# VincentGourbin/ltx-video-swift-mlx

Hardware: AMD Instinct MI355X
Metric: DiT denoise steps/sec + VAE decode ms, 768x512x25 distilled (higher is better)
Workload: dtype bf16; 1 GPU; distilled 8-step schedule, 768x512x25 -> latent 4x16x24 (1536 tokens), 1024 text keys, CFG off, batch 1 per GPU, 48-layer DiT bf16 weights (random init); text_keys=1024, parallelism=replica x1 (one sample per GPU, no data-path collective)

## Files before the change

### include/ltxhip.h

```cpp
#ifndef LTXHIP_H
#define LTXHIP_H

#include <stddef.h>
#include <stdint.h>

#ifdef __cplusplus
extern "C" {
#endif

typedef struct ltx_ctx ltx_ctx;

typedef enum ltx_status {
    LTX_OK = 0,
    LTX_ERR_MODEL_NOT_LOADED = 1,
    LTX_ERR_INVALID_CONFIGURATION = 2,
    LTX_ERR_INSUFFICIENT_MEMORY = 3,
    LTX_ERR_WEIGHT_LOADING_FAILED = 4,
    LTX_ERR_GENERATION_FAILED = 5,
    LTX_ERR_GENERATION_CANCELLED = 6,
    LTX_ERR_INVALID_FRAME_COUNT = 7,
    LTX_ERR_INVALID_DIMENSIONS = 8,
    LTX_ERR_FILE_NOT_FOUND = 9,
    LTX_ERR_INVALID_LORA = 10,
    LTX_ERR_HIP = 11
// ... 333 lines not shown
                                const float* noise, int tile, int overlap, int root, float* frames_out, long frames_cap,
                                int* n_frames_out);

int ltx_prof_enable(ltx_ctx* ctx, int on);
int ltx_prof_collect(ltx_ctx* ctx, int kind, double* total_ms, long* launches, double* work, int reset);

int ltx_op_gemm_bf16(ltx_ctx* ctx, const uint16_t* A, long lda, const uint16_t* B, long ldb, const float* bias, int M,
                     int N, int K, int act, int tile_cfg, float* out_f32, long ld_f32, uint16_t* out_bf16,
                     long ld_bf16);
int ltx_op_gemm_q8(ltx_ctx* ctx, const uint16_t* A, long lda, const uint8_t* codes, const uint16_t* scales, const uint16_t* biases,
                   const float* bias, int M, int N, int K, int split_k, int via_scratch, int tile_cfg, float* out_f32, long ld_f32);
int ltx_op_value_projection_t(ltx_ctx* ctx, const uint16_t* X, long ldx, int tokens, const uint16_t* W, const float* bias, int out_features,
                              int in_features, uint16_t* vt, long ldvt);
int ltx_op_qkv_projection(ltx_ctx* ctx, const uint16_t* X, long ldx, int rows, int rows_per_batch, const uint16_t* Wqk, const float* bqk,
                          const uint16_t* Wv, const float* bv, int D, int K, uint16_t* qk_out, long ld_qk, uint16_t* vt_out, long ldvt,
                          int fused);
int ltx_op_gemm_bf16_gated_residual(ltx_ctx* ctx, const uint16_t* A, long lda, const uint16_t* B, long ldb,
                                    const float* bias, const float* gate, float gate_scalar, int M, int N, int K,
                                    float* x, long ldx, uint16_t* mirror_bf16, long ld_mirror);
int ltx_op_gemm_bf16_gated_residual_norm(ltx_ctx* ctx, const uint16_t* A, long lda, const uint16_t* B, long ldb,
                                         const float* bias, const float* gate, float gate_scalar, int M, int N, int K,
                                         float* x, long ldx, const float* scale, const float* shift, float eps,
                                         uint16_t* xn, long ldxn, int fused);
int ltx_op_gemv_f32(ltx_ctx* ctx, const float* a, long lda, const uint16_t* W, long ldw, const float* bias, float* out,
                    long ldo, int M, int N, int K, int in_act);
typedef struct ltx_gemv_job {
    const float* a;
    long lda;
    const uint16_t* W;
    long ldw;
    const float* bias;
    float* out;
    long ldo;
    int N;
    int K;
    int in_act;
} ltx_gemv_job;
int ltx_op_gemv_group(ltx_ctx* ctx, const ltx_gemv_job* jobs, int n_jobs, int M);
int ltx_op_attention(ltx_ctx* ctx, const uint16_t* Q, const uint16_t* K, const uint16_t* Vt, long ldvt,
                     const float* bias, int B, int H, int Tq, int Tk, float scale, uint16_t* O);
int ltx_attention_key_splits(int B, int H, int Tq, int Tk);
int ltx_op_attention_hd(ltx_ctx* ctx, const uint16_t* Q, const uint16_t* K, const uint16_t* Vt, long ldvt, const float* bias, int B, int H,
                        int Tq, int Tk, int head_dim, float scale, uint16_t* O);
int ltx_attention_hd_workgroup_queries(int B, int H, int Tq, int head_dim);
int ltx_op_norm_mod(ltx_ctx* ctx, const float* x, const float* scale, const float* shift, int rows, int D,
                    int norm_kind, float eps, int round_norm_bf16, uint16_t* out);
// ... 27 lines not shown
```

### ltx-video-swift-mlx_amd/__init__.py

```python
import contextlib
import ctypes as C

import numpy as np

from . import _lib
from ._lib import (ALLGATHER_FN, DIST_ID_BYTES, SHARD_CFG, SHARD_NONE, SHARD_SEQUENCE, ConnectorConfig, PROGRESS_CB, DenoiseOptions,
                   DualBlockConfig, DualDenoiseArgs, DualForwardArgs, DualModelConfig, DualModelForwardArgs, DualStepJob, GemvJob,
                   LTXError, NormMod2Job, TransformerConfig, lib)

__version__ = lib.ltx_version().decode()


def _check(rc, ctx=None):
    if rc != 0:
        msg = lib.ltx_last_error(ctx).decode(errors="replace") if True else ""
        raise LTXError(rc, msg)


def default_dual_block_config(**overrides):
    cfg = DualBlockConfig()
    lib.ltx_dual_block_config_default(C.byref(cfg))
    o = dict(overrides)
    if "video_heads" in o:
        o.setdefault("video_dim", o["video_heads"] * 128)
    if "audio_heads" in o:
        o.setdefault("audio_dim", o["audio_heads"] * 64)
    if "video_dim" in o:
        o.setdefault("video_context_dim", o["video_dim"])
    if "audio_dim" in o:
        o.setdefault("audio_context_dim", o["audio_dim"])
# ... 1008 lines not shown
```

### ltx-video-swift-mlx_amd/_lib.py

```python
import ctypes as C
import os

_HERE = os.path.dirname(os.path.abspath(__file__))
SO_PATH = os.environ.get("LTX_LIB") or os.path.join(_HERE, "csrc", "build", "libltxhip.so")


class LTXError(RuntimeError):

    NAMES = {
        1: "modelNotLoaded", 2: "invalidConfiguration", 3: "insufficientMemory", 4: "weightLoadingFailed",
        5: "generationFailed", 6: "generationCancelled", 7: "invalidFrameCount", 8: "invalidDimensions",
        9: "fileNotFound", 10: "invalidLoRA", 11: "hipError",
    }

    def __init__(self, code, message):
        self.code = int(code)
        self.case = self.NAMES.get(self.code, "unknown")
        super().__init__(f"LTXError.{self.case}: {message}")


class DenoiseOptions(C.Structure):

    _fields_ = [("struct_size", C.c_uint32), ("cfg_scale", C.c_float), ("guidance_rescale", C.c_float), ("stg_scale", C.c_float),
                ("stg_blocks", C.POINTER(C.c_int)), ("n_stg_blocks", C.c_int), ("ge_gamma", C.c_float),
# ... 22 lines not shown
        ("timestep_scale_multiplier", C.c_float), ("norm_eps", C.c_float),
    ]


class DualBlockConfig(C.Structure):

    _fields_ = [("num_layers", C.c_int), ("video_heads", C.c_int), ("video_dim", C.c_int), ("audio_heads", C.c_int), ("audio_dim", C.c_int),
                ("video_context_dim", C.c_int), ("audio_context_dim", C.c_int), ("rope_theta", C.c_float), ("max_pos", C.c_int * 3),
                ("audio_max_pos", C.c_int), ("fps", C.c_float), ("norm_eps", C.c_float)]


class DualForwardArgs(C.Structure):

    _fields_ = [("struct_size", C.c_uint32), ("B", C.c_int), ("F", C.c_int), ("H", C.c_int), ("W", C.c_int), ("T_a", C.c_int), ("S", C.c_int),
                ("x_video", C.c_void_p), ("x_audio", C.c_void_p), ("context_video", C.c_void_p), ("context_audio", C.c_void_p),
                ("key_bias_video", C.c_void_p), ("key_bias_audio", C.c_void_p), ("temb_video", C.c_void_p), ("temb_audio", C.c_void_p),
                ("cross_video_ss", C.c_void_p), ("cross_audio_ss", C.c_void_p), ("phase_mask", C.c_uint32)]


class GemvJob(C.Structure):

    _fields_ = [("a", C.c_void_p), ("lda", C.c_long), ("W", C.c_void_p), ("ldw", C.c_long), ("bias", C.c_void_p), ("out", C.c_void_p),
                ("ldo", C.c_long), ("N", C.c_int), ("K", C.c_int), ("in_act", C.c_int)]


class DualModelConfig(C.Structure):

    _fields_ = [("blocks", DualBlockConfig), ("in_channels", C.c_int), ("out_channels", C.c_int), ("audio_in_channels", C.c_int),
                ("audio_out_channels", C.c_int), ("caption_channels", C.c_int), ("timestep_scale_multiplier", C.c_float)]


class DualModelForwardArgs(C.Structure):

    _fields_ = [("struct_size", C.c_uint32), ("B", C.c_int), ("F", C.c_int), ("H", C.c_int), ("W", C.c_int), ("T_a", C.c_int), ("S", C.c_int),
                ("video_latent", C.c_void_p), ("audio_latent", C.c_void_p), ("video_context", C.c_void_p), ("audio_context", C.c_void_p),
                ("video_timesteps", C.c_void_p), ("audio_timesteps", C.c_void_p), ("video_mask", C.c_void_p), ("audio_mask", C.c_void_p),
                ("video_velocity", C.c_void_p), ("audio_velocity", C.c_void_p), ("ungrouped", C.c_int), ("text_cache", C.c_int)]


class NormMod2Job(C.Structure):

    _fields_ = [("x", C.c_void_p), ("ldx", C.c_long), ("scale0", C.c_void_p), ("shift0", C.c_void_p), ("scale1", C.c_void_p),
                ("shift1", C.c_void_p), ("mod_bstride", C.c_long), ("rows_per_batch", C.c_int), ("out0", C.c_void_p), ("out1", C.c_void_p),
                ("ldo", C.c_long), ("rows", C.c_int), ("D", C.c_int)]


# ... 143 lines not shown
    "ltx_audio_decode": (_i, [_vp, _vp, _i, _vp]),
    "ltx_audio_decode_dev": (_i, [_vp, _vp, _i, _vp]),
    "ltx_audio_latent_frames": (_i, [_i, _f]),
    "ltx_audio_mel_frames": (_i, [_i]),
    "ltx_audio_sample_count": (_l, [_i]),
    "ltx_audio_sample_rate": (_i, []),
    "ltx_write_wav": (_i, [C.c_char_p, _vp, _l, _i, _f]),
    "ltx_audio_positions": (_i, [_i, _vp]),
    "ltx_video_temporal_positions": (_i, [_i, _i, _i, _f, _vp]),
    "ltx_rope_tables_positions": (_i, [_vp, _i, _i, _f, _i, _vp, _vp]),
    "ltx_attn_module_init_synthetic": (_i, [_vp, _i, _i, _i, _i, _u64]),
    "ltx_attn_module_load": (_i, [_vp, _i, C.c_char_p, C.c_char_p, _i]),
    "ltx_attn_module_unload": (_i, [_vp, _i]),
    "ltx_attn_module_export_param": (_l, [_vp, _i, C.c_char_p, _vp, _l]),
    "ltx_attn_module_forward_dev": (_i, [_vp, _i, _vp, _vp, _i, _i, _i, _i, _vp, _vp, _i, _vp, _vp, _i, _vp, _vp]),
    "ltx_dual_block_config_default": (None, [C.POINTER(DualBlockConfig)]),
    "ltx_dual_blocks_init_synthetic": (_i, [_vp, C.POINTER(DualBlockConfig), _u64]),
    "ltx_dual_blocks_load": (_i, [_vp, C.c_char_p, C.POINTER(DualBlockConfig), _i, _i]),
    "ltx_dual_blocks_unload": (_i, [_vp]),
    "ltx_dual_blocks_export_param": (_l, [_vp, C.c_char_p, _vp, _l]),
    "ltx_dual_blocks_forward_dev": (_i, [_vp, C.POINTER(DualForwardArgs)]),
    "ltx_op_norm_mod2": (_i, [_vp, C.POINTER(NormMod2Job), C.POINTER(NormMod2Job), _f]),
    "ltx_op_gemv_group": (_i, [_vp, C.POINTER(GemvJob), _i, _i]),
    "ltx_dual_model_config_default": (None, [C.POINTER(DualModelConfig)]),
    "ltx_dual_model_init_synthetic": (_i, [_vp, C.POINTER(DualModelConfig), _u64]),
    "ltx_dual_model_load": (_i, [_vp, C.c_char_p, C.POINTER(DualModelConfig)]),
    "ltx_dual_model_unload": (_i, [_vp]),
    "ltx_dual_model_export_param": (_l, [_vp, C.c_char_p, _vp, _l]),
    "ltx_dual_model_forward_dev": (_i, [_vp, C.POINTER(DualModelForwardArgs)]),
    "ltx_dual_model_embed_dev": (_i, [_vp, _vp, _vp, _i, _i, _vp, _vp, _vp, _vp, _vp, _vp]),
    "ltx_dual_model_prepare_text_dev": (_i, [_vp, _vp, _vp, _vp, _vp, _i, _i]),
    "ltx_dual_model_text_cache_info": (_i, [_vp, _ip, _ip, C.POINTER(_l), C.POINTER(_l)]),
    "ltx_op_dual_step": (_i, [_vp, C.POINTER(DualStepJob), C.POINTER(DualStepJob), _f, _f]),
    "ltx_dual_denoise_dev": (_i, [_vp, C.POINTER(DualDenoiseArgs), PROGRESS_CB, _vp]),
    "ltx_dual_denoise": (_i, [_vp, C.POINTER(DualDenoiseArgs), PROGRESS_CB, _vp]),
    "ltx_op_attention_hd": (_i, [_vp, _vp, _vp, _vp, _l, _vp, _i, _i, _i, _i, _i, _f, _vp]),
    "ltx_attention_hd_workgroup_queries": (_i, [_i, _i, _i, _i]),
    "ltx_op_qknorm_rope_hd": (_i, [_vp, _vp, _l, _vp, _vp, _vp, _i, _i, _i, _i, _f, _f, _vp]),
    "ltx_op_conv1d": (_i, [_vp, _vp, _i, _i, _vp, _vp, _i, _i, _i, _i, _vp, _i, _i, _vp, _i, _f, _vp]),
    "ltx_op_conv_transpose1d": (_i, [_vp, _vp, _i, _i, _vp, _vp, _i, _i, _i, _i, _i, _vp, _i, _f, _vp]),
    "ltx_op_conv2d_causal": (_i, [_vp, _vp, _i, _i, _i, _vp, _vp, _i, _i, _i, _vp, _i, _vp, _vp]),
    "ltx_op_fill_normal_bf16": (_i, [_vp, _vp, _l, _u64, _f, _f]),
    "ltx_op_fill_normal_f32": (_i, [_vp, _vp, _l, _u64, _f, _f]),
}

for _name, (_res, _args) in SIGNATURES.items():
# ... 6 lines not shown
```

### ltx-video-swift-mlx_amd/csrc/abi_hooks.cpp

```cpp
#include <vector>

#include "abi_internal.h"
#include "attention.h"
#include "audio.h"
#include "elementwise.h"
#include "gemm.h"
#include "linear_ops.h"

namespace {

void op_workspace(ltx_ctx* ctx, size_t bytes) {
    if (ctx->op_ws.ensure(bytes)) HIP_CHECK(hipStreamSynchronize(ctx->stream));
}

const bf16_t* audio_halo_operand(ltx_ctx* ctx, const uint16_t* x, int Cin, int lines, int width, int pitch, size_t first, size_t total) {
    const size_t row = (size_t)Cin * 2;
    ctx->audio_op[0].ensure(total * row);
    char* base = ctx->audio_op[0].as<char>();
    if (pitch == width) {
        HIP_CHECK(hipMemsetAsync(base, 0, first * row, ctx->stream));
        const size_t end = first + (size_t)lines * width;
        HIP_CHECK(hipMemsetAsync(base + end * row, 0, (total - end) * row, ctx->stream));
        HIP_CHECK(hipMemcpyAsync(base + first * row, x, (size_t)lines * width * row, hipMemcpyDeviceToDevice, ctx->stream));
    } else {
// ... 151 lines not shown
                                         float* x, long ldx, const float* scale, const float* shift, float eps,
                                         uint16_t* xn, long ldxn, int fused) {
    return with_ctx(ctx, [&] {
        LTX_REQUIRE(A && B && x && scale && shift && xn, "ltx_op_gemm_bf16_gated_residual_norm: null argument");
        GemmArgs g;
        g.A = A; g.lda = lda; g.B = B; g.ldb = ldb; g.M = M; g.N = N; g.K = K;
        g.ep.bias_n = bias;
        g.ep.out_f32 = x; g.ep.ld_f32 = ldx;
        g.ep.resid = 1;
        g.ep.gate = gate; g.ep.gate_bstride = 0; g.ep.rows_per_batch = M; g.ep.gate_scalar = gate_scalar;
        op_workspace(ctx, (size_t)2 * M * N * 4);
        g.split_k = 0;
        g.split_ws = ctx->op_ws.as<float>();
        g.split_ws_elems = (long)(ctx->op_ws.bytes / 4);
        NormAfter na;
        na.scale = scale; na.shift = shift; na.mod_bstride = 0; na.rows_per_batch = M;
        na.out = xn; na.ldo = ldxn; na.eps = eps; na.norm_kind = LTX_NORM_RMS;
        if (fused) {
            launch_gemm_bf16(g, ctx->stream, &na);
        } else {
            launch_gemm_bf16(g, ctx->stream);
            launch_norm_mod(x, ldx, scale, shift, 0, M, xn, ldxn, M, N, LTX_NORM_RMS, eps, 0, ctx->stream);
        }
    });
}

int ltx_op_gemv_f32(ltx_ctx* ctx, const float* a, long lda, const uint16_t* W, long ldw, const float* bias, float* out,
                    long ldo, int M, int N, int K, int in_act) {
    return with_ctx(ctx, [&] { launch_gemv_f32(a, lda, W, ldw, bias, out, ldo, M, N, K, in_act, ctx->stream); });
}

int ltx_op_gemv_group(ltx_ctx* ctx, const ltx_gemv_job* jobs, int n_jobs, int M) {
    return with_ctx(ctx, [&] {
        LTX_REQUIRE(jobs && n_jobs >= 1 && n_jobs <= 8, "ltx_op_gemv_group: %d jobs out of range (1..8)", n_jobs);
        GemvJob g[8];
        for (int j = 0; j < n_jobs; ++j) {
            const ltx_gemv_job& q = jobs[j];
            g[j].a = q.a; g[j].lda = q.lda; g[j].W = q.W; g[j].ldw = q.ldw; g[j].bias = q.bias;
            g[j].out = q.out; g[j].ldo = q.ldo; g[j].N = q.N; g[j].K = q.K; g[j].in_act = q.in_act;
        }
        launch_gemv_group(g, n_jobs, M, ctx->stream);
    });
}

int ltx_op_conv3d(ltx_ctx* ctx, const uint16_t* x, int F, int H, int W, int Cin, const uint16_t* w, const float* bias,
                  int Cout, int causal, float* out) {
// ... 257 lines not shown
```

### ltx-video-swift-mlx_amd/csrc/gemm_asm_tiles.inc

```
namespace {

LTX_DEVFN int asm_src_offset(int lane, int wave, long ld) {
    const int srow = lane >> 3, pch = lane & 7;
    const int row0 = wave * 8 + srow;
    return (row0 * (int)ld + ((pch ^ ((row0 >> 1) & 7)) << 3)) * 2;
}
LTX_DEVFN uint32_t asm_src_stride(long ld) { return (uint32_t)(32 * ld * 2); }

struct AsmLane {
    int ao, bo;
    uint32_t sa, sb;
    uint32_t wlds;
    int fa0, fa1, fb0, fb1;
};
template <int WM, int WCOL, int A_BYTES>
LTX_DEVFN AsmLane asm_lane(int lane, int wave, int wr, int wc, long lda, long ldb) {
    AsmLane l;
    l.ao = asm_src_offset(lane, wave, lda);
    l.bo = asm_src_offset(lane, wave, ldb);
    l.sa = asm_src_stride(lda);
    l.sb = asm_src_stride(ldb);
    l.wlds = (uint32_t)wave * 1024u;
    const int frow = lane & 15, fsw = (lane >> 1) & 7;
    const int foff0 = frow * ROW_BYTES + ((((lane >> 4) + 0) ^ fsw) << 4);
    const int foff1 = frow * ROW_BYTES + ((((lane >> 4) + 4) ^ fsw) << 4);
    const int a_wave_off = (wr * WM) * ROW_BYTES, b_wave_off = 2 * A_BYTES + (wc * WCOL) * ROW_BYTES;
    l.fa0 = a_wave_off + foff0, l.fa1 = a_wave_off + foff1, l.fb0 = b_wave_off + foff0, l.fb1 = b_wave_off + foff1;
    return l;
}

struct AsmBufDesc {
    uint32_t lo, hi, rec;
};
LTX_DEVFN AsmBufDesc asm_buf_desc(const bf16_t* p, int rows, long ld, long kelems) {
    return {(uint32_t)(uintptr_t)p, (uint32_t)((uintptr_t)p >> 32), (uint32_t)(((long)(rows - 1) * ld + kelems) * 2)};
}

template <int WN>
LTX_DEVFN int asm_scratch_lane(int lane) { return (((lane >> 4) * 4) * WN + (lane & 15)) * 4; }

#if defined(DTL_STAMPS) || defined(QKV_STAMPS) || defined(TALL_STAMPS)
LTX_DEVFN unsigned long long* asm_stamp_slot(int wave) { return (blockIdx.x == 7) ? &g_gemm_stamps[wave][0] : &g_gemm_stamps[4][0]; }
#endif

LTX_DEVFN f32x4 asm_column_bias(const float* bias_n, int gn) { return bias_n ? *(const f32x4*)(bias_n + gn) : f32x4{0.f, 0.f, 0.f, 0.f}; }

template <bool BIAS_M>
LTX_DEVFN f32x4 asm_activate(const GemmEpilogue& ep, f32x4 v, int gm) {
    if constexpr (BIAS_M) {
        if (ep.bias_m) {
            const float bm = ep.bias_m[gm];
            v += f32x4{bm, bm, bm, bm};
        }
    }
    if (ep.act == LTX_ACT_GELU_TANH) {
#pragma unroll
        for (int e = 0; e < 4; ++e) v[e] = gelu_tanh(v[e]);
    } else if (ep.act == LTX_ACT_SILU) {
#pragma unroll
        for (int e = 0; e < 4; ++e) v[e] = silu_f(v[e]);
    }
    if (ep.round_bf16) {
#pragma unroll
        for (int e = 0; e < 4; ++e) v[e] = bf16_to_f32(f32_to_bf16(v[e]));
    }
// ... 8 lines not shown
LTX_DEVFN void asm_store(const GemmEpilogue& ep, int gm, int gn, const f32x4& v) {
    if (ep.out_f32) *(f32x4*)(ep.out_f32 + (long)gm * ep.ld_f32 + gn) = v;
    if (ep.out_bf16) asm_store_bf16(ep.out_bf16, ep.ld_bf16, gm, gn, v);
}
template <bool BIAS_M>
struct AsmPlainStore {
    const GemmEpilogue& ep;
    LTX_DEVFN void operator()(int gm, int gn, f32x4 v) const { asm_store(ep, gm, gn, asm_activate<BIAS_M>(ep, v, gm)); }
};

template <int WN>
struct AsmGroup {
    static constexpr int LPR = WN / 4, RPI = 64 / LPR, NITG = 32 / RPI;
};
template <int WN, class Put>
LTX_DEVFN void asm_store_group(const float* scr, int lane, int gm0, int gn, const f32x4& bias, Put&& put) {
    using G = AsmGroup<WN>;
    f32x4 vv[G::NITG];
#pragma unroll
    for (int it = 0; it < G::NITG; ++it) vv[it] = *(const f32x4*)(scr + (it * G::RPI + lane / G::LPR) * WN + (lane % G::LPR) * 4);
#pragma unroll
    for (int it = 0; it < G::NITG; ++it) put(gm0 + it * G::RPI + lane / G::LPR, gn, vv[it] + bias);
    asm volatile("s_waitcnt lgkmcnt(0)" ::: "memory");
}

__global__ __launch_bounds__(256, 1) void gemm_bf16_kernel_dtl(const GemmArgs g) {
    extern __shared__ __attribute__((aligned(16))) char smem[];
    constexpr int BM = 192, BN = 256, WGN = 2;
    constexpr int WM = 96, WN = 128;
    const int tid = threadIdx.x;
    const int lane = tid & 63;
    const int wave = __builtin_amdgcn_readfirstlane(tid >> 6);
    const int wr = wave / WGN, wc = wave % WGN;
    const int tiles_m = g.M / BM;
    const int bid = xcd_remap(blockIdx.x, gridDim.x);
    int tm, tn;
    tile_coords(g, bid, tiles_m, BN, tm, tn);
    const int m0 = tm * BM, n0 = tn * BN;
    int kt0 = 0, nkt = g.K / BK;
    if (g.split_k > 1) {
        const int z = blockIdx.y;
        kt0 = (int)((long)nkt * z / g.split_k);
        nkt = (int)((long)nkt * (z + 1) / g.split_k) - kt0;
    }
    const AsmLane l = asm_lane<WM, WN, BM * ROW_BYTES>(lane, wave, wr, wc, g.lda, g.ldb);
    const AsmBufDesc a = asm_buf_desc(g.A + (long)m0 * g.lda + (long)kt0 * BK, BM, g.lda, (long)nkt * BK);
    const AsmBufDesc b = asm_buf_desc(g.B + (long)n0 * g.ldb + (long)kt0 * BK, BN, g.ldb, (long)nkt * BK);
    const uint32_t nk = (uint32_t)nkt;
#ifdef DTL_STAMPS
    unsigned long long* dbg = asm_stamp_slot(wave);
#endif
    asm volatile(
#ifdef DTL_STAMPS
#include "gemm_dtl_192x256_stamps.inc"
#else
#include "gemm_dtl_192x256.inc"
#endif
        :
        : [alo] "s"(a.lo), [ahi] "s"(a.hi), [arec] "s"(a.rec), [blo] "s"(b.lo), [bhi] "s"(b.hi), [brec] "s"(b.rec), [nk] "s"(nk), [sa] "s"(l.sa),
          [sb] "s"(l.sb), [wlds] "s"(l.wlds), [ao] "v"(l.ao), [bo] "v"(l.bo), [fa0] "v"(l.fa0), [fa1] "v"(l.fa1), [fb0] "v"(l.fb0), [fb1] "v"(l.fb1)
#ifdef DTL_STAMPS
          , [dbg] "s"(dbg)
#endif
        :
#include "gemm_dtl_192x256_clobbers.inc"
    );
    __syncthreads();
    constexpr int LPR = AsmGroup<WN>::LPR, RPI = AsmGroup<WN>::RPI, NITG = AsmGroup<WN>::NITG;
    float* scr = (float*)(smem + wave * (32 * WN * 4));
    const unsigned scr_lane = (unsigned)(wave * (32 * WN * 4) + asm_scratch_lane<WN>(lane));
    const int gn = n0 + wc * WN + (lane % LPR) * 4;
    if (g.split_k > 1) {
        float* ws = g.split_ws + (long)blockIdx.y * g.M * g.N;
        bf16_t* wsb = (bf16_t*)g.split_ws + (long)blockIdx.y * g.M * g.N;
        static_for<0, 3>([&](auto grp_c) {
            constexpr int grp = decltype(grp_c)::value;
#include "gemm_asm_192x256_dump.inc"
#pragma unroll 4
            for (int it = 0; it < 32 / RPI; ++it) {
                const int row = it * RPI + lane / LPR;
                const f32x4 v = *(const f32x4*)(scr + row * WN + (lane % LPR) * 4);
                if (g.split_bf16) asm_store_bf16(wsb, g.N, m0 + wr * WM + grp * 32 + row, gn, v);
                else *(f32x4*)(ws + (long)(m0 + wr * WM + grp * 32 + row) * g.N + gn) = v;
            }
            asm volatile("s_waitcnt lgkmcnt(0)" ::: "memory");
        });
        return;
    }
    const GemmEpilogue& ep = g.ep;
    const f32x4 bias = asm_column_bias(ep.bias_n, gn);
    if (ep.resid) {
        const float* rbase = ep.resid_src ? ep.resid_src : ep.out_f32;
        const long rld = ep.resid_src ? ep.ld_resid : ep.ld_f32;
        const int row_lo = m0 + wr * WM, row_hi = row_lo + WM - 1;
        const bool gate_uniform = ep.gate && !ep.gate_rowmap && row_lo / ep.rows_per_batch == row_hi / ep.rows_per_batch;
        f32x4 gtu = f32x4{ep.gate_scalar, ep.gate_scalar, ep.gate_scalar, ep.gate_scalar};
        if (gate_uniform) gtu = *(const f32x4*)(ep.gate + (long)(row_lo / ep.rows_per_batch) * ep.gate_bstride + gn);
        f32x4 rs[2][NITG];
        auto fetch = [&](auto grp_c, auto buf_c) {
            constexpr int grp = decltype(grp_c)::value, buf = decltype(buf_c)::value;
#pragma unroll
            for (int it = 0; it < NITG; ++it) rs[buf][it] = *(const f32x4*)(rbase + (long)(m0 + wr * WM + grp * 32 + it * RPI + lane / LPR) * rld + gn);
        };
        fetch(std::integral_constant<int, 0>{}, std::integral_constant<int, 0>{});
        static_for<0, 3>([&](auto grp_c) {
            constexpr int grp = decltype(grp_c)::value;
            constexpr int buf = grp & 1;
            if constexpr (grp + 1 < 3) fetch(std::integral_constant<int, grp + 1>{}, std::integral_constant<int, (grp + 1) & 1>{});
#include "gemm_asm_192x256_dump.inc"
            static_for<0, 2>([&](auto half_c) {
                constexpr int half = decltype(half_c)::value;
                f32x4 vv[NITG / 2];
#pragma unroll
                for (int i2 = 0; i2 < NITG / 2; ++i2) vv[i2] = *(const f32x4*)(scr + ((half * (NITG / 2) + i2) * RPI + lane / LPR) * WN + (lane % LPR) * 4);
#pragma unroll
                for (int i2 = 0; i2 < NITG / 2; ++i2) {
                    const int it = half * (NITG / 2) + i2;
                    const int gm = m0 + wr * WM + grp * 32 + it * RPI + lane / LPR;
                    f32x4 v = asm_activate<true>(ep, vv[i2] + bias, gm);
                    f32x4 gt = gtu;
                    if (ep.gate && !gate_uniform)
                        gt = *(const f32x4*)(ep.gate + (long)(ep.gate_rowmap ? ep.gate_rowmap[gm] : gm / ep.rows_per_batch) * ep.gate_bstride + gn);
#pragma unroll
                    for (int e = 0; e < 4; ++e) v[e] = rs[buf][it][e] + gt[e] * v[e];
                    asm_store(ep, gm, gn, v);
                }
            });
            asm volatile("s_waitcnt lgkmcnt(0)" ::: "memory");
        });
        return;
    }
    static_for<0, 3>([&](auto grp_c) {
        constexpr int grp = decltype(grp_c)::value;
#include "gemm_asm_192x256_dump.inc"
        asm_store_group<WN>(scr, lane, m0 + wr * WM + grp * 32, gn, bias, AsmPlainStore<true>{ep});
    });
}

__global__ __launch_bounds__(256, 1) void gemm_bf16_kernel_qkv(const GemmQkvArgs g) {
    extern __shared__ __attribute__((aligned(16))) char smem[];
    constexpr int BM = 192, WM = 96, WNQ = 128, WNV = 64;
    const int tid = threadIdx.x;
    const int lane = tid & 63;
    const int wave = __builtin_amdgcn_readfirstlane(tid >> 6);
    const int wr = wave / 2, wc = wave % 2;
    const int tiles_m = g.M / BM;
    const int bid = xcd_remap(blockIdx.x, gridDim.x);
    int tm, tn;
    tile_coords(g.group_m, g.Nqk / 256, bid, tiles_m, tm, tn);
    const int m0 = tm * BM;
    const AsmLane l = asm_lane<WM, WNQ + WNV, BM * ROW_BYTES>(lane, wave, wr, wc, g.ldx, g.ldwqk);
    const int vo = asm_src_offset(lane, wave, g.ldwv);
    const uint32_t sv = asm_src_stride(g.ldwv);
    const AsmBufDesc a = asm_buf_desc(g.X + (long)m0 * g.ldx, BM, g.ldx, g.K);
    const AsmBufDesc b = asm_buf_desc(g.Wqk + (long)tn * 256 * g.ldwqk, 256, g.ldwqk, g.K);
    const AsmBufDesc v = asm_buf_desc(g.Wv + (long)tn * 128 * g.ldwv, 128, g.ldwv, g.K);
    const uint32_t nk = (uint32_t)(g.K / BK);
    constexpr int SPILL0 = 4 * 32 * WNQ * 4;
    const int sp = SPILL0 + wave * 8192 + lane * 16;
#ifdef QKV_STAMPS
    unsigned long long* dbg = asm_stamp_slot(wave);
#endif
    asm volatile(
#ifdef QKV_STAMPS
#include "gemm_qkv_192x384_stamps.inc"
#else
#include "gemm_qkv_192x384.inc"
#endif
        :
        : [alo] "s"(a.lo), [ahi] "s"(a.hi), [arec] "s"(a.rec), [blo] "s"(b.lo), [bhi] "s"(b.hi), [brec] "s"(b.rec), [vlo] "s"(v.lo), [vhi] "s"(v.hi),
          [vrec] "s"(v.rec), [nk] "s"(nk), [sa] "s"(l.sa), [sb] "s"(l.sb), [sv] "s"(sv), [wlds] "s"(l.wlds), [ao] "v"(l.ao), [bo] "v"(l.bo), [vo] "v"(vo),
          [fa0] "v"(l.fa0), [fa1] "v"(l.fa1), [fb0] "v"(l.fb0), [fb1] "v"(l.fb1), [sp] "v"(sp)
#ifdef QKV_STAMPS
          , [dbg] "s"(dbg)
#endif
        :
#include "gemm_qkv_192x384_clobbers.inc"
    );
    {
        const int bi = m0 / g.rows_per_batch;
        const int tok0 = m0 - bi * g.rows_per_batch + wr * WM + (lane >> 4) * 4;
        const int d0 = tn * 128 + wc * WNV + (lane & 15);
        bf16_t* vbase = g.vt + (long)bi * g.vt_bstride + tok0;
        float bv[4];
#pragma unroll
        for (int nv = 0; nv < 4; ++nv) bv[nv] = g.bias_v ? g.bias_v[d0 + nv * 16] : 0.f;
        static_for<0, 24>([&](auto vf_c) {
            constexpr int vf = decltype(vf_c)::value;
            constexpr int mi = vf / 4, nv = vf % 4;
            float f0, f1, f2, f3;
            if constexpr (vf < 16) {
#include "gemm_qkv_192x384_vread.inc"
            } else {
                const f32x4 t = *(const f32x4*)(smem + SPILL0 + wave * 8192 + (vf - 16) * 1024 + lane * 16);
                f0 = t[0], f1 = t[1], f2 = t[2], f3 = t[3];
            }
            const float bn = bv[nv];
            uint2 pk;
            pk.x = pack_bf16x2(f0 + bn, f1 + bn);
            pk.y = pack_bf16x2(f2 + bn, f3 + bn);
            *(uint2*)(vbase + (long)(d0 + nv * 16) * g.ldvt + mi * 16) = pk;
        });
    }
    constexpr int WN = WNQ;
    float* scr = (float*)(smem + wave * (32 * WN * 4));
    const unsigned scr_lane = (unsigned)(wave * (32 * WN * 4) + asm_scratch_lane<WN>(lane));
    const int gn = tn * 256 + wc * WN + (lane % AsmGroup<WN>::LPR) * 4;
    const f32x4 bias = asm_column_bias(g.bias_qk, gn);
    static_for<0, 3>([&](auto grp_c) {
        constexpr int grp = decltype(grp_c)::value;
#include "gemm_asm_192x256_dump.inc"
        asm_store_group<WN>(scr, lane, m0 + wr * WM + grp * 32, gn, bias,
                            [&](int gm, int gn_, const f32x4& val) { asm_store_bf16(g.qk, g.ld_qk, gm, gn_, val); });
    });
}

__global__ __launch_bounds__(256, 1) void gemm_bf16_kernel_tall(const GemmArgs g) {
    extern __shared__ __attribute__((aligned(16))) char smem[];
    constexpr int BM = 384, BN = 256, WGN = 2;
    constexpr int WM = 192, WN = 128;
    constexpr int WAVE_LDS = 2 * 32 * WN * 4;
    const int tid = threadIdx.x;
    const int lane = tid & 63;
    const int wave = __builtin_amdgcn_readfirstlane(tid >> 6);
    const int wr = wave / WGN, wc = wave % WGN;
    const int tiles_m = g.M / BM;
    const int bid = xcd_remap(blockIdx.x, gridDim.x);
    int tm, tn;
    tile_coords(g, bid, tiles_m, BN, tm, tn);
    const int m0 = tm * BM, n0 = tn * BN;
    const int nkt = g.K / BK;
    const AsmLane l = asm_lane<WM, WN, BM * ROW_BYTES>(lane, wave, wr, wc, g.lda, g.ldb);
    const AsmBufDesc a = asm_buf_desc(g.A + (long)m0 * g.lda, BM, g.lda, (long)nkt * BK);
    const AsmBufDesc b = asm_buf_desc(g.B + (long)n0 * g.ldb, BN, g.ldb, (long)nkt * BK);
    const uint32_t nk = (uint32_t)nkt;
    const int sp = wave * WAVE_LDS + asm_scratch_lane<WN>(lane);
#ifdef TALL_STAMPS
    unsigned long long* dbg = asm_stamp_slot(wave);
#endif
    asm volatile(
#ifdef TALL_STAMPS
#include "gemm_tall_384x256_stamps.inc"
#else
#include "gemm_tall_384x256.inc"
#endif
        :
        : [alo] "s"(a.lo), [ahi] "s"(a.hi), [arec] "s"(a.rec), [blo] "s"(b.lo), [bhi] "s"(b.hi), [brec] "s"(b.rec), [nk] "s"(nk), [sa] "s"(l.sa),
          [sb] "s"(l.sb), [wlds] "s"(l.wlds), [ao] "v"(l.ao), [bo] "v"(l.bo), [fa0] "v"(l.fa0), [fa1] "v"(l.fa1), [fb0] "v"(l.fb0), [fb1] "v"(l.fb1), [sp] "v"(sp)
#ifdef TALL_STAMPS
          , [dbg] "s"(dbg)
#endif
        :
#include "gemm_tall_384x256_clobbers.inc"
    );
    const unsigned scr_lane = (unsigned)(wave * WAVE_LDS + asm_scratch_lane<WN>(lane));
    const int gn = n0 + wc * WN + (lane % AsmGroup<WN>::LPR) * 4;
    const GemmEpilogue& ep = g.ep;
    const f32x4 bias = asm_column_bias(ep.bias_n, gn);
    static_for<0, 6>([&](auto ord_c) {
        constexpr int grp = (decltype(ord_c)::value + 4) % 6;
        const float* scr = (const float*)(smem + wave * WAVE_LDS + (grp == 5 ? 32 * WN * 4 : 0));
        if constexpr (grp < 4) {
#include "gemm_tall_384x256_dump.inc"
        }
        asm_store_group<WN>(scr, lane, m0 + wr * WM + grp * 32, gn, bias, AsmPlainStore<false>{ep});
    });
}

}

template <auto KERNEL, int SMEM, class Args>
static void launch_asm_tile(dim3 grid, const Args& a, hipStream_t stream) {
    static PerDeviceOnce attr_set;
    attr_set.run([&] { HIP_CHECK(hipFuncSetAttribute((const void*)KERNEL, hipFuncAttributeMaxDynamicSharedMemorySize, SMEM)); });
    hipLaunchKernelGGL(KERNEL, grid, dim3(256), SMEM, stream, a);
    HIP_CHECK(hipGetLastError());
}

static bool gemm_dtl_takes(const GemmArgs& a) {
    return !a.conv && a.M % 192 == 0 && a.N % 256 == 0 && a.K % 64 == 0 && a.K >= 64 && !a.ep.d2s && !a.ep.out_bf16_t &&
           a.lda % 8 == 0 && a.ldb % 8 == 0 && !a.ep.pn_out && !a.ep.clip01 && a.tile_count == 0 && a.win_rows == 0 &&
           (a.split_k <= 1 || (a.split_ws && a.split_k <= a.K / 64 && (long)a.split_k * a.M * a.N <= a.split_ws_elems));
}
static void launch_dtl(const GemmArgs& a, const GemmOpts& o, hipStream_t stream, const NormAfter* na = nullptr) {
    LTX_REQUIRE(gemm_dtl_takes(a), "gemm: the 192x256 kernel needs a dense A.B^T with M %% 192 == 0, N %% 256 == 0, K %% 64 == 0 (M=%d N=%d K=%d)",
                a.M, a.N, a.K);
    constexpr int smem = (2 * 192 + 3 * 256) * ROW_BYTES;
    launch_asm_tile<gemm_bf16_kernel_dtl, smem>(dim3((a.M / 192) * (a.N / 256), a.split_k > 1 ? a.split_k : 1), a, stream);
    if (a.split_k > 1) {
// ... 57 lines not shown
```

Before: 30.68 steps/s.

## Specialise asm GEMM epilogues with compile-time store variants and strength-reduced row pointers

Adds templated row-store functors that precompute output row pointers and step them by constant strides. A runtime variant selector dispatches common epilogues (plain bf16, GELU-tanh bf16, f32, f32+bf16 mirror, gated residual fast paths) to compile-time specialised loops, so the generic per-element epilogue branching is skipped. The same store path is applied to the DTL, QKV, tall and split-K partial kernels. It also adds optional epilogue cycle stamps and a standalone ltx_op_gemm_tile ABI entry for testing tiles, at the cost of more code and instantiations.

Result: faster. 31.19 steps/s (median of 6 runs) (+1.7%).

```diff
diff --git a/include/ltxhip.h b/include/ltxhip.h
--- a/include/ltxhip.h
+++ b/include/ltxhip.h
@@ -379,6 +379,34 @@
                                          const float* bias, const float* gate, float gate_scalar, int M, int N, int K,
                                          float* x, long ldx, const float* scale, const float* shift, float eps,
                                          uint16_t* xn, long ldxn, int fused);
+typedef struct ltx_gemm_tile_launch {
+    uint32_t struct_size;
+    int tile_cfg;
+    const uint16_t* A;
+    long lda;
+    const uint16_t* B;
+    long ldb;
+    int M, N, K;
+    int split_k;
+    int split_bf16;
+    int act;
+    int round_bf16;
+    int resid;
+    const float* bias_n;
+    const float* bias_m;
+    float* out_f32;
+    long ld_f32;
+    uint16_t* out_bf16;
+    long ld_bf16;
+    const float* resid_src;
+    long ld_resid;
+    const float* gate;
+    long gate_bstride;
+    const int32_t* gate_rowmap;
+    int rows_per_batch;
+    float gate_scalar;
+} ltx_gemm_tile_launch;
+int ltx_op_gemm_tile(ltx_ctx* ctx, const ltx_gemm_tile_launch* launch);
 int ltx_op_gemv_f32(ltx_ctx* ctx, const float* a, long lda, const uint16_t* W, long ldw, const float* bias, float* out,
                     long ldo, int M, int N, int K, int in_act);
 typedef struct ltx_gemv_job {
diff --git a/ltx-video-swift-mlx_amd/__init__.py b/ltx-video-swift-mlx_amd/__init__.py
--- a/ltx-video-swift-mlx_amd/__init__.py
+++ b/ltx-video-swift-mlx_amd/__init__.py
@@ -5,7 +5,7 @@
 
 from . import _lib
 from ._lib import (ALLGATHER_FN, DIST_ID_BYTES, SHARD_CFG, SHARD_NONE, SHARD_SEQUENCE, ConnectorConfig, PROGRESS_CB, DenoiseOptions,
-                   DualBlockConfig, DualDenoiseArgs, DualForwardArgs, DualModelConfig, DualModelForwardArgs, DualStepJob, GemvJob,
+                   DualBlockConfig, DualDenoiseArgs, DualForwardArgs, DualModelConfig, DualModelForwardArgs, DualStepJob, GemmTileLaunch, GemvJob,
                    LTXError, NormMod2Job, TransformerConfig, lib)
 
 __version__ = lib.ltx_version().decode()
diff --git a/ltx-video-swift-mlx_amd/_lib.py b/ltx-video-swift-mlx_amd/_lib.py
--- a/ltx-video-swift-mlx_amd/_lib.py
+++ b/ltx-video-swift-mlx_amd/_lib.py
@@ -68,6 +68,16 @@
 
     _fields_ = [("a", C.c_void_p), ("lda", C.c_long), ("W", C.c_void_p), ("ldw", C.c_long), ("bias", C.c_void_p), ("out", C.c_void_p),
                 ("ldo", C.c_long), ("N", C.c_int), ("K", C.c_int), ("in_act", C.c_int)]
+
+
+class GemmTileLaunch(C.Structure):
+
+    _fields_ = [("struct_size", C.c_uint32), ("tile_cfg", C.c_int), ("A", C.c_void_p), ("lda", C.c_long), ("B", C.c_void_p), ("ldb", C.c_long),
+                ("M", C.c_int), ("N", C.c_int), ("K", C.c_int), ("split_k", C.c_int), ("split_bf16", C.c_int), ("act", C.c_int),
+                ("round_bf16", C.c_int), ("resid", C.c_int), ("bias_n", C.c_void_p), ("bias_m", C.c_void_p), ("out_f32", C.c_void_p),
+                ("ld_f32", C.c_long), ("out_bf16", C.c_void_p), ("ld_bf16", C.c_long), ("resid_src", C.c_void_p), ("ld_resid", C.c_long),
+                ("gate", C.c_void_p), ("gate_bstride", C.c_long), ("gate_rowmap", C.c_void_p), ("rows_per_batch", C.c_int),
+                ("gate_scalar", C.c_float)]
 
 
 class DualModelConfig(C.Structure):
@@ -257,6 +267,7 @@
     "ltx_dual_blocks_forward_dev": (_i, [_vp, C.POINTER(DualForwardArgs)]),
     "ltx_op_norm_mod2": (_i, [_vp, C.POINTER(NormMod2Job), C.POINTER(NormMod2Job), _f]),
     "ltx_op_gemv_group": (_i, [_vp, C.POINTER(GemvJob), _i, _i]),
+    "ltx_op_gemm_tile": (_i, [_vp, C.POINTER(GemmTileLaunch)]),
     "ltx_dual_model_config_default": (None, [C.POINTER(DualModelConfig)]),
     "ltx_dual_model_init_synthetic": (_i, [_vp, C.POINTER(DualModelConfig), _u64]),
     "ltx_dual_model_load": (_i, [_vp, C.c_char_p, C.POINTER(DualModelConfig)]),
diff --git a/ltx-video-swift-mlx_amd/csrc/abi_hooks.cpp b/ltx-video-swift-mlx_amd/csrc/abi_hooks.cpp
--- a/ltx-video-swift-mlx_amd/csrc/abi_hooks.cpp
+++ b/ltx-video-swift-mlx_amd/csrc/abi_hooks.cpp
@@ -197,6 +197,30 @@
             launch_gemm_bf16(g, ctx->stream);
             launch_norm_mod(x, ldx, scale, shift, 0, M, xn, ldxn, M, N, LTX_NORM_RMS, eps, 0, ctx->stream);
         }
+    });
+}
+
+int ltx_op_gemm_tile(ltx_ctx* ctx, const ltx_gemm_tile_launch* l) {
+    return with_ctx(ctx, [&] {
+        LTX_REQUIRE(l && l->struct_size == sizeof(ltx_gemm_tile_launch), "ltx_op_gemm_tile: null argument or a struct_size of another ABI");
+        LTX_REQUIRE(l->tile_cfg == 75 || l->tile_cfg == 76, "ltx_op_gemm_tile: tile_cfg %d is neither 75 (192x256) nor 76 (384x256)", l->tile_cfg);
+        LTX_REQUIRE(l->A && l->B && l->split_k >= 1, "ltx_op_gemm_tile: null operand or split_k < 1");
+        GemmArgs g;
+        g.A = l->A; g.lda = l->lda; g.B = l->B; g.ldb = l->ldb; g.M = l->M; g.N = l->N; g.K = l->K;
+        GemmEpilogue& e = g.ep;
+        e.bias_n = l->bias_n; e.bias_m = l->bias_m; e.act = l->act; e.round_bf16 = l->round_bf16;
+        e.out_f32 = l->out_f32; e.ld_f32 = l->ld_f32; e.out_bf16 = l->out_bf16; e.ld_bf16 = l->ld_bf16;
+        e.resid = l->resid; e.resid_src = l->resid_src; e.ld_resid = l->ld_resid;
+        e.gate = l->gate; e.gate_bstride = l->gate_bstride; e.gate_rowmap = l->gate_rowmap; e.gate_scalar = l->gate_scalar;
+        e.rows_per_batch = l->rows_per_batch > 0 ? l->rows_per_batch : l->M;
+        if (l->split_k > 1) {
+            g.split_k = l->split_k;
+            g.split_bf16 = l->split_bf16;
+            op_workspace(ctx, (size_t)g.split_k * l->M * l->N * 4);
+            g.split_ws = ctx->op_ws.as<float>();
+            g.split_ws_elems = (long)(ctx->op_ws.bytes / 4);
+        }
+        launch_gemm_bf16_cfg(g, l->tile_cfg, ctx->stream);
     });
 }
 
diff --git a/ltx-video-swift-mlx_amd/csrc/gemm_asm_tiles.inc b/ltx-video-swift-mlx_amd/csrc/gemm_asm_tiles.inc
--- a/ltx-video-swift-mlx_amd/csrc/gemm_asm_tiles.inc
+++ b/ltx-video-swift-mlx_amd/csrc/gemm_asm_tiles.inc
@@ -41,6 +41,20 @@
 
 #if defined(DTL_STAMPS) || defined(QKV_STAMPS) || defined(TALL_STAMPS)
 LTX_DEVFN unsigned long long* asm_stamp_slot(int wave) { return (blockIdx.x == 7) ? &g_gemm_stamps[wave][0] : &g_gemm_stamps[4][0]; }
+__device__ unsigned long long g_gemm_epi_stamps[5][16];
+#define ASM_EPI_STAMPS unsigned long long epi_ts[16] = {}
+#define ASM_EPI_STAMP(i) epi_ts[i] = __builtin_readcyclecounter()
+#define ASM_EPI_STAMPS_FLUSH(n)                                                               \
+    do {                                                                                      \
+        asm volatile("s_waitcnt vmcnt(0)" ::: "memory");                                      \
+        ASM_EPI_STAMP(n);                                                                     \
+        if (lane == 0)                                                                        \
+            for (int i_ = 0; i_ <= (n); ++i_) g_gemm_epi_stamps[blockIdx.x == 7 ? wave : 4][i_] = epi_ts[i_]; \
+    } while (0)
+#else
+#define ASM_EPI_STAMPS
+#define ASM_EPI_STAMP(i)
+#define ASM_EPI_STAMPS_FLUSH(n)
 #endif
 
 LTX_DEVFN f32x4 asm_column_bias(const float* bias_n, int gn) { return bias_n ? *(const f32x4*)(bias_n + gn) : f32x4{0.f, 0.f, 0.f, 0.f}; }
@@ -95,6 +109,79 @@
 #pragma unroll
     for (int it = 0; it < G::NITG; ++it) put(gm0 + it * G::RPI + lane / G::LPR, gn, vv[it] + bias);
     asm volatile("s_waitcnt lgkmcnt(0)" ::: "memory");
+}
+
+typedef __attribute__((ext_vector_type(2))) float f32x2;
+typedef __attribute__((ext_vector_type(2))) __bf16 bf16x2_t;
+
+LTX_DEVFN uint2 asm_pack_bf16x4(const f32x4& v) {
+    const bf16x2_t lo = __builtin_convertvector(f32x2{v[0], v[1]}, bf16x2_t);
+    const bf16x2_t hi = __builtin_convertvector(f32x2{v[2], v[3]}, bf16x2_t);
+    return uint2{__builtin_bit_cast(uint32_t, lo), __builtin_bit_cast(uint32_t, hi)};
+}
+LTX_DEVFN f32x2 asm_gelu_tanh2(f32x2 x) {
+    const float c0 = -2.0f * 0.7978845608028654f * 1.4426950408889634f;
+    const float c1 = c0 * 0.044715f;
+    const f32x2 t = x * __builtin_elementwise_fma(f32x2{c1, c1}, x * x, f32x2{c0, c0});
+    const f32x2 d = f32x2{1.0f, 1.0f} + f32x2{__builtin_amdgcn_exp2f(t[0]), __builtin_amdgcn_exp2f(t[1])};
+    return x * f32x2{__builtin_amdgcn_rcpf(d[0]), __builtin_amdgcn_rcpf(d[1])};
+}
+
+enum { ASM_OUT_BF16 = 1, ASM_OUT_F32 = 2 };
+template <int ACT, int OUTS, bool BIAS>
+struct AsmRowStore {
+    bf16_t* pb;
+    float* pf;
+    long sb, sf;
+    f32x4 bias;
+    LTX_DEVFN AsmRowStore after(int steps) const { return {pb + steps * sb, pf + steps * sf, sb, sf, bias}; }
+    LTX_DEVFN void operator()(f32x4 v) {
+        if constexpr (BIAS) v += bias;
+        if constexpr (ACT == LTX_ACT_GELU_TANH) {
+            const f32x2 lo = asm_gelu_tanh2(f32x2{v[0], v[1]}), hi = asm_gelu_tanh2(f32x2{v[2], v[3]});
+            v = f32x4{lo[0], lo[1], hi[0], hi[1]};
+        }
+        if constexpr ((OUTS & ASM_OUT_F32) != 0) {
+            *(f32x4*)pf = v;
+            pf += sf;
+        }
+        if constexpr ((OUTS & ASM_OUT_BF16) != 0) {
+            *(uint2*)pb = asm_pack_bf16x4(v);
+            pb += sb;
+        }
+    }
+};
+template <int WN, int ACT, int OUTS, bool BIAS>
+LTX_DEVFN AsmRowStore<ACT, OUTS, BIAS> asm_row_store(bf16_t* out_bf16, long ld_bf16, float* out_f32, long ld_f32, int lane, int row0, int gn, const f32x4& bias) {
+    using G = AsmGroup<WN>;
+    const int row = row0 + lane / G::LPR;
+    return {out_bf16 + (long)row * ld_bf16 + gn, out_f32 + (long)row * ld_f32 + gn, G::RPI * ld_bf16, G::RPI * ld_f32, bias};
+}
+template <int WN, class Put>
+LTX_DEVFN void asm_store_rows(const float* scr, int lane, Put put) {
+    using G = AsmGroup<WN>;
+    f32x4 vv[G::NITG];
+#pragma unroll
+    for (int it = 0; it < G::NITG; ++it) vv[it] = *(const f32x4*)(scr + (it * G::RPI + lane / G::LPR) * WN + (lane % G::LPR) * 4);
+#pragma unroll
+    for (int it = 0; it < G::NITG; ++it) put(vv[it]);
+    asm volatile("s_waitcnt lgkmcnt(0)" ::: "memory");
+}
+LTX_DEVFN int asm_plain_variant(const GemmEpilogue& ep) {
+    if (ep.bias_m || (ep.round_bf16 && ep.out_f32)) return 0;
+    if (ep.act == LTX_ACT_NONE) return ep.out_f32 ? (ep.out_bf16 ? 4 : 3) : 1;
+    if (ep.act == LTX_ACT_GELU_TANH && !ep.out_f32) return 2;
+    return 0;
+}
+template <class Body>
+LTX_DEVFN bool asm_plain_dispatch(int variant, Body&& body) {
+    using std::integral_constant;
+    if (variant == 1) body(integral_constant<int, LTX_ACT_NONE>{}, integral_constant<int, ASM_OUT_BF16>{});
+    else if (variant == 2) body(integral_constant<int, LTX_ACT_GELU_TANH>{}, integral_constant<int, ASM_OUT_BF16>{});
+    else if (variant == 3) body(integral_constant<int, LTX_ACT_NONE>{}, integral_constant<int, ASM_OUT_F32>{});
+    else if (variant == 4) body(integral_constant<int, LTX_ACT_NONE>{}, integral_constant<int, ASM_OUT_F32 | ASM_OUT_BF16>{});
+    else return false;
+    return true;
 }
 
 __global__ __launch_bounds__(256, 1) void gemm_bf16_kernel_dtl(const GemmArgs g) {
@@ -139,6 +226,8 @@
 #include "gemm_dtl_192x256_clobbers.inc"
     );
     __syncthreads();
+    ASM_EPI_STAMPS;
+    ASM_EPI_STAMP(0);
     constexpr int LPR = AsmGroup<WN>::LPR, RPI = AsmGroup<WN>::RPI, NITG = AsmGroup<WN>::NITG;
     float* scr = (float*)(smem + wave * (32 * WN * 4));
     const unsigned scr_lane = (unsigned)(wave * (32 * WN * 4) + asm_scratch_lane<WN>(lane));
@@ -146,18 +235,20 @@
     if (g.split_k > 1) {
         float* ws = g.split_ws + (long)blockIdx.y * g.M * g.N;
         bf16_t* wsb = (bf16_t*)g.split_ws + (long)blockIdx.y * g.M * g.N;
-        static_for<0, 3>([&](auto grp_c) {
-            constexpr int grp = decltype(grp_c)::value;
+        auto partial = [&](auto outs_c) {
+            constexpr int outs = decltype(outs_c)::value;
+            const auto st = asm_row_store<WN, LTX_ACT_NONE, outs, false>(wsb, g.N, ws, g.N, lane, m0 + wr * WM, gn, f32x4{});
+            static_for<0, 3>([&](auto grp_c) {
+                constexpr int grp = decltype(grp_c)::value;
 #include "gemm_asm_192x256_dump.inc"
-#pragma unroll 4
-            for (int it = 0; it < 32 / RPI; ++it) {
-                const int row = it * RPI + lane / LPR;
-                const f32x4 v = *(const f32x4*)(scr + row * WN + (lane % LPR) * 4);
-                if (g.split_bf16) asm_store_bf16(wsb, g.N, m0 + wr * WM + grp * 32 + row, gn, v);
-                else *(f32x4*)(ws + (long)(m0 + wr * WM + grp * 32 + row) * g.N + gn) = v;
-            }
-            asm volatile("s_waitcnt lgkmcnt(0)" ::: "memory");
-        });
+                ASM_EPI_STAMP(1 + 2 * grp);
+                asm_store_rows<WN>(scr, lane, st.after(grp * NITG));
+                ASM_EPI_STAMP(2 + 2 * grp);
+            });
+        };
+        if (g.split_bf16) partial(std::integral_constant<int, ASM_OUT_BF16>{});
+        else partial(std::integral_constant<int, ASM_OUT_F32>{});
+        ASM_EPI_STAMPS_FLUSH(7);
         return;
     }
     const GemmEpilogue& ep = g.ep;
@@ -169,45 +260,80 @@
         const bool gate_uniform = ep.gate && !ep.gate_rowmap && row_lo / ep.rows_per_batch == row_hi / ep.rows_per_batch;
         f32x4 gtu = f32x4{ep.gate_scalar, ep.gate_scalar, ep.gate_scalar, ep.gate_scalar};
         if (gate_uniform) gtu = *(const f32x4*)(ep.gate + (long)(row_lo / ep.rows_per_batch) * ep.gate_bstride + gn);
-        f32x4 rs[2][NITG];
-        auto fetch = [&](auto grp_c, auto buf_c) {
-            constexpr int grp = decltype(grp_c)::value, buf = decltype(buf_c)::value;
-#pragma unroll
-            for (int it = 0; it < NITG; ++it) rs[buf][it] = *(const f32x4*)(rbase + (long)(m0 + wr * WM + grp * 32 + it * RPI + lane / LPR) * rld + gn);
+        auto resid_body = [&](auto fast_c, auto mirror_c, auto gate_rows_c) {
+            constexpr bool FAST = decltype(fast_c)::value, MIRROR = decltype(mirror_c)::value, GATE_ROWS = decltype(gate_rows_c)::value;
+            const float* rp = rbase + (long)(row_lo + lane / LPR) * rld + gn;
+            const long rstep = RPI * rld;
+            auto st = asm_row_store<WN, LTX_ACT_NONE, ASM_OUT_F32 | (MIRROR ? ASM_OUT_BF16 : 0), false>(ep.out_bf16, ep.ld_bf16, ep.out_f32, ep.ld_f32, lane, row_lo,
+                                                                                                     gn, f32x4{});
+            f32x4 rs[2][NITG];
+            auto fetch = [&](auto grp_c, auto buf_c) {
+                constexpr int grp = decltype(grp_c)::value, buf = decltype(buf_c)::value;
+#pragma unroll
+                for (int it = 0; it < NITG; ++it) rs[buf][it] = *(const f32x4*)(rp + (grp * NITG + it) * rstep);
+            };
+            fetch(std::integral_constant<int, 0>{}, std::integral_constant<int, 0>{});
+            static_for<0, 3>([&](auto grp_c) {
+                constexpr int grp = decltype(grp_c)::value;
+                constexpr int buf = grp & 1;
+                if constexpr (grp + 1 < 3) fetch(std::integral_constant<int, grp + 1>{}, std::integral_constant<int, (grp + 1) & 1>{});
+#include "gemm_asm_192x256_dump.inc"
+                static_for<0, 2>([&](auto half_c) {
+                    constexpr int half = decltype(half_c)::value;
+                    f32x4 vv[NITG / 2];
+#pragma unroll
+                    for (int i2 = 0; i2 < NITG / 2; ++i2) vv[i2] = *(const f32x4*)(scr + ((half * (NITG / 2) + i2) * RPI + lane / LPR) * WN + (lane % LPR) * 4);
+#pragma unroll
+                    for (int i2 = 0; i2 < NITG / 2; ++i2) {
+                        const int it = half * (NITG / 2) + i2;
+                        const int gm = row_lo + grp * 32 + it * RPI + lane / LPR;
+                        f32x4 v = vv[i2] + bias;
+                        if constexpr (!FAST) v = asm_activate<true>(ep, v, gm);
+                        f32x4 gt = gtu;
+                        if constexpr (!FAST) {
+                            if (ep.gate && !gate_uniform)
+                                gt = *(const f32x4*)(ep.gate + (long)(ep.gate_rowmap ? ep.gate_rowmap[gm] : gm / ep.rows_per_batch) * ep.gate_bstride + gn);
+                        } else if constexpr (GATE_ROWS) {
+                            gt = *(const f32x4*)(ep.gate + (long)(ep.gate_rowmap ? ep.gate_rowmap[gm] : gm / ep.rows_per_batch) * ep.gate_bstride + gn);
+                        }
+#pragma unroll
+                        for (int e = 0; e < 4; ++e) v[e] = rs[buf][it][e] + gt[e] * v[e];
+                        if constexpr (FAST) st(v);
+                        else asm_store(ep, gm, gn, v);
+                    }
+                });
+                asm volatile("s_waitcnt lgkmcnt(0)" ::: "memory");
+            });
         };
-        fetch(std::integral_constant<int, 0>{}, std::integral_constant<int, 0>{});
+        using std::false_type;
+        using std::true_type;
+        const bool fast = !ep.bias_m && ep.act == LTX_ACT_NONE && !ep.round_bf16 && ep.out_f32;
+        const bool gate_rows = ep.gate && !gate_uniform;
+        if (!fast) resid_body(false_type{}, false_type{}, false_type{});
+        else if (gate_rows) ep.out_bf16 ? resid_body(true_type{}, true_type{}, true_type{}) : resid_body(true_type{}, false_type{}, true_type{});
+        else ep.out_bf16 ? resid_body(true_type{}, true_type{}, false_type{}) : resid_body(true_type{}, false_type{}, false_type{});
+        return;
+    }
+    const bool specialised = asm_plain_dispatch(__builtin_amdgcn_readfirstlane(asm_plain_variant(ep)), [&](auto act_c, auto outs_c) {
+        const auto st = asm_row_store<WN, decltype(act_c)::value, decltype(outs_c)::value, true>(ep.out_bf16, ep.ld_bf16, ep.out_f32, ep.ld_f32, lane,
+                                                                                                 m0 + wr * WM, gn, bias);
         static_for<0, 3>([&](auto grp_c) {
             constexpr int grp = decltype(grp_c)::value;
-            constexpr int buf = grp & 1;
-            if constexpr (grp + 1 < 3) fetch(std::integral_constant<int, grp + 1>{}, std::integral_constant<int, (grp + 1) & 1>{});
 #include "gemm_asm_192x256_dump.inc"
-            static_for<0, 2>([&](auto half_c) {
-                constexpr int half = decltype(half_c)::value;
-                f32x4 vv[NITG / 2];
-#pragma unroll
-                for (int i2 = 0; i2 < NITG / 2; ++i2) vv[i2] = *(const f32x4*)(scr + ((half * (NITG / 2) + i2) * RPI + lane / LPR) * WN + (lane % LPR) * 4);
-#pragma unroll
-                for (int i2 = 0; i2 < NITG / 2; ++i2) {
-                    const int it = half * (NITG / 2) + i2;
-                    const int gm = m0 + wr * WM + grp * 32 + it * RPI + lane / LPR;
-                    f32x4 v = asm_activate<true>(ep, vv[i2] + bias, gm);
-                    f32x4 gt = gtu;
-                    if (ep.gate && !gate_uniform)
-                        gt = *(const f32x4*)(ep.gate + (long)(ep.gate_rowmap ? ep.gate_rowmap[gm] : gm / ep.rows_per_batch) * ep.gate_bstride + gn);
-#pragma unroll
-                    for (int e = 0; e < 4; ++e) v[e] = rs[buf][it][e] + gt[e] * v[e];
-                    asm_store(ep, gm, gn, v);
-                }
-            });
-            asm volatile("s_waitcnt lgkmcnt(0)" ::: "memory");
+            ASM_EPI_STAMP(1 + 2 * grp);
+            asm_store_rows<WN>(scr, lane, st.after(grp * NITG));
+            ASM_EPI_STAMP(2 + 2 * grp);
         });
-        return;
-    }
-    static_for<0, 3>([&](auto grp_c) {
-        constexpr int grp = decltype(grp_c)::value;
+    });
+    if (!specialised)
+        static_for<0, 3>([&](auto grp_c) {
+            constexpr int grp = decltype(grp_c)::value;
 #include "gemm_asm_192x256_dump.inc"
-        asm_store_group<WN>(scr, lane, m0 + wr * WM + grp * 32, gn, bias, AsmPlainStore<true>{ep});
-    });
+            ASM_EPI_STAMP(1 + 2 * grp);
+            asm_store_group<WN>(scr, lane, m0 + wr * WM + grp * 32, gn, bias, AsmPlainStore<true>{ep});
+            ASM_EPI_STAMP(2 + 2 * grp);
+        });
+    ASM_EPI_STAMPS_FLUSH(7);
 }
 
 __global__ __launch_bounds__(256, 1) void gemm_bf16_kernel_qkv(const GemmQkvArgs g) {
@@ -250,14 +376,20 @@
         :
 #include "gemm_qkv_192x384_clobbers.inc"
     );
+    ASM_EPI_STAMPS;
+    ASM_EPI_STAMP(0);
     {
         const int bi = m0 / g.rows_per_batch;
         const int tok0 = m0 - bi * g.rows_per_batch + wr * WM + (lane >> 4) * 4;
         const int d0 = tn * 128 + wc * WNV + (lane & 15);
         bf16_t* vbase = g.vt + (long)bi * g.vt_bstride + tok0;
         float bv[4];
-#pragma unroll
-        for (int nv = 0; nv < 4; ++nv) bv[nv] = g.bias_v ? g.bias_v[d0 + nv * 16] : 0.f;
+        bf16_t* vrow[4];
+#pragma unroll
+        for (int nv = 0; nv < 4; ++nv) {
+            bv[nv] = g.bias_v ? g.bias_v[d0 + nv * 16] : 0.f;
+            vrow[nv] = vbase + (long)(d0 + nv * 16) * g.ldvt;
+        }
         static_for<0, 24>([&](auto vf_c) {
             constexpr int vf = decltype(vf_c)::value;
             constexpr int mi = vf / 4, nv = vf % 4;
@@ -269,23 +401,24 @@
                 f0 = t[0], f1 = t[1], f2 = t[2], f3 = t[3];
             }
             const float bn = bv[nv];
-            uint2 pk;
-            pk.x = pack_bf16x2(f0 + bn, f1 + bn);
-            pk.y = pack_bf16x2(f2 + bn, f3 + bn);
-            *(uint2*)(vbase + (long)(d0 + nv * 16) * g.ldvt + mi * 16) = pk;
+            *(uint2*)(vrow[nv] + mi * 16) = asm_pack_bf16x4(f32x4{f0 + bn, f1 + bn, f2 + bn, f3 + bn});
         });
     }
+    ASM_EPI_STAMP(1);
     constexpr int WN = WNQ;
     float* scr = (float*)(smem + wave * (32 * WN * 4));
     const unsigned scr_lane = (unsigned)(wave * (32 * WN * 4) + asm_scratch_lane<WN>(lane));
     const int gn = tn * 256 + wc * WN + (lane % AsmGroup<WN>::LPR) * 4;
     const f32x4 bias = asm_column_bias(g.bias_qk, gn);
+    const auto qk_store = asm_row_store<WN, LTX_ACT_NONE, ASM_OUT_BF16, true>(g.qk, g.ld_qk, nullptr, 0, lane, m0 + wr * WM, gn, bias);
     static_for<0, 3>([&](auto grp_c) {
         constexpr int grp = decltype(grp_c)::value;
 #include "gemm_asm_192x256_dump.inc"
-        asm_store_group<WN>(scr, lane, m0 + wr * WM + grp * 32, gn, bias,
-                            [&](int gm, int gn_, const f32x4& val) { asm_store_bf16(g.qk, g.ld_qk, gm, gn_, val); });
+        ASM_EPI_STAMP(2 + 2 * grp);
+        asm_store_rows<WN>(scr, lane, qk_store.after(grp * AsmGroup<WN>::NITG));
+        ASM_EPI_STAMP(3 + 2 * grp);
     });
+    ASM_EPI_STAMPS_FLUSH(8);
 }
 
 __global__ __launch_bounds__(256, 1) void gemm_bf16_kernel_tall(const GemmArgs g) {
@@ -326,18 +459,38 @@
         :
 #include "gemm_tall_384x256_clobbers.inc"
     );
+    ASM_EPI_STAMPS;
+    ASM_EPI_STAMP(0);
     const unsigned scr_lane = (unsigned)(wave * WAVE_LDS + asm_scratch_lane<WN>(lane));
     const int gn = n0 + wc * WN + (lane % AsmGroup<WN>::LPR) * 4;
     const GemmEpilogue& ep = g.ep;
     const f32x4 bias = asm_column_bias(ep.bias_n, gn);
-    static_for<0, 6>([&](auto ord_c) {
-        constexpr int grp = (decltype(ord_c)::value + 4) % 6;
-        const float* scr = (const float*)(smem + wave * WAVE_LDS + (grp == 5 ? 32 * WN * 4 : 0));
-        if constexpr (grp < 4) {
+    const bool specialised = asm_plain_dispatch(__builtin_amdgcn_readfirstlane(asm_plain_variant(ep)), [&](auto act_c, auto outs_c) {
+        const auto st = asm_row_store<WN, decltype(act_c)::value, decltype(outs_c)::value, true>(ep.out_bf16, ep.ld_bf16, ep.out_f32, ep.ld_f32, lane,
+                                                                                                 m0 + wr * WM, gn, bias);
+        static_for<0, 6>([&](auto ord_c) {
+            constexpr int grp = (decltype(ord_c)::value + 4) % 6;
+            const float* scr = (const float*)(smem + wave * WAVE_LDS + (grp == 5 ? 32 * WN * 4 : 0));
+            if constexpr (grp < 4) {
 #include "gemm_tall_384x256_dump.inc"
-        }
-        asm_store_group<WN>(scr, lane, m0 + wr * WM + grp * 32, gn, bias, AsmPlainStore<false>{ep});
+            }
+            ASM_EPI_STAMP(1 + 2 * decltype(ord_c)::value);
+            asm_store_rows<WN>(scr, lane, st.after(grp * AsmGroup<WN>::NITG));
+            ASM_EPI_STAMP(2 + 2 * decltype(ord_c)::value);
+        });
     });
+    if (!specialised)
+        static_for<0, 6>([&](auto ord_c) {
+            constexpr int grp = (decltype(ord_c)::value + 4) % 6;
+            const float* scr = (const float*)(smem + wave * WAVE_LDS + (grp == 5 ? 32 * WN * 4 : 0));
+            if constexpr (grp < 4) {
+#include "gemm_tall_384x256_dump.inc"
+            }
+            ASM_EPI_STAMP(1 + 2 * decltype(ord_c)::value);
+            asm_store_group<WN>(scr, lane, m0 + wr * WM + grp * 32, gn, bias, AsmPlainStore<false>{ep});
+            ASM_EPI_STAMP(2 + 2 * decltype(ord_c)::value);
+        });
+    ASM_EPI_STAMPS_FLUSH(13);
 }
 
 }
```
